# rayanirban/DiffSplitting

Hardware: AMD Instinct MI355X
Metric: sampled images/sec (2000-step 128x128 SR3) (higher is better)
Workload: dtype bf16; 1 GPU; sr_sr3_16_128: GaussianDiffusion.p_sample_loop, 16->128 SR3 UNet (97.8M params), T=2000 linear schedule; one step = UNet forward + posterior update of the batch; batch_per_gpu=16, global_batch=16, image=128x128x3, sample_steps=2000, parallelism=1 independent replicas, final RCCL all-gather, hipgraph=True, streams=1, noise=device Philox4x32-10, weights=random-init, seed 0

## Files before the change

### diffsplitting_amd/csrc/dsx_conv.hip

```cpp
#include "dsx_conv_variants.h"
#include <mutex>

namespace dsx {

int conv_chunk_multiple(int ks) { return conv_cpg(ks); }

static_assert(kIndex.unique, "kVariants: two rows share a key, or a key is outside key_slot's ranges");

static constexpr bool variants_consistent() {
  for (const ConvVariant& a : kVariants) {
    const bool big = a.family != FAM_MFMA || (a.ks == 3 && a.cpg == 2);
    if (a.lds_cap != (big ? kLdsMax : kLdsDefault) || a.block != (a.family == FAM_MFMA ? 256 : 512)) return false;
    for (const ConvVariant& b : kVariants) {
      if (a.tile == b.tile && (a.MB * a.WM != b.MB * b.WM || a.WN * a.NB != b.WN * b.NB)) return false;
      if (a.tile == b.tile && a.family == b.family && (a.WM != b.WM || a.fuses_stats != b.fuses_stats)) return false;
    }
  }
  return true;
}
static_assert(variants_consistent(), "kVariants: wrong LDS limit / block size, or two layouts for one tile");

ConvTileInfo conv_tile_info(int tile, bool ws) {
  for (const ConvVariant& v : kVariants)
    if (v.family == (ws ? FAM_WS : FAM_MFMA) && v.tile == tile) return {32 * v.MB * v.WM, 32 * v.WN * v.NB, v.WM, v.fuses_stats};
  return {0, 0, 0, false};
}

namespace lds_row_was {
constexpr int banked(int rb, int tw_log2) {
  if (tw_log2 == 4) rb = (rb + 255) & ~255;
  else if (tw_log2 == 3) { rb = (rb + 127) & ~127; if (((rb >> 7) & 1) == 0) rb += 128; }
  return rb;
}
constexpr int plain(int ks, int stride, int tw_log2) {
  const int rb = ((((1 << tw_log2) - 1) * stride + ks) * (64 * conv_cpg(ks) + 16) + 15) & ~15;
  return (ks == 1 || stride != 1) ? rb : banked(rb, tw_log2);
}
constexpr int g2(int tw_log2) { return banked(((((1 << tw_log2) - 1) + 3) * (64 * 2 + 16) + 15) & ~15, tw_log2); }
constexpr int c3x3(int tw_log2, int cpg) { return banked(((((1 << tw_log2) - 1) + 3) * (64 * cpg + 16) + 15) & ~15, tw_log2); }
constexpr int c4_1x1(int tw_log2) { return (((1 << tw_log2) * (64 * 4 + 16)) + 15) & ~15; }
constexpr bool same() {
  for (int tw = 0; tw <= 4; ++tw) {
    for (int cpg = 1; cpg <= 4; cpg *= 2)
      if (conv_lds_row(3, 1, tw, cpg) != c3x3(tw, cpg)) return false;
    if (conv_lds_row(3, 1, tw, 1) != plain(3, 1, tw) || conv_lds_row(3, 1, tw, 2) != g2(tw)) return false;
    if (conv_lds_row(3, 2, tw, 1) != plain(3, 2, tw)) return false;
    if (conv_lds_row(1, 1, tw, 2) != plain(1, 1, tw) || conv_lds_row(1, 1, tw, 4) != c4_1x1(tw)) return false;
  }
  return true;
}
static_assert(same(), "conv_lds_row changed a row pitch");
}

hipError_t conv_init() {
  static std::mutex mu;
  static bool done = false;
  std::lock_guard<std::mutex> lock(mu);
  if (done) return hipSuccess;
  for (const ConvVariant& v : kVariants) {
    const hipError_t e = hipFuncSetAttribute((const void*)v.kern, hipFuncAttributeMaxDynamicSharedMemorySize, v.lds_cap);
    if (e != hipSuccess) return e;
  }
  done = true;
  return hipSuccess;
}

}
```

### diffsplitting_amd/csrc/dsx_conv_direct.hip

```cpp
#include "dsx_conv_common.h"

namespace dsx {

template <typename DT>
__global__ __launch_bounds__(256) void k_conv_first(const ConvArgs a) {
  constexpr bool F32 = sizeof(DT) == 4;
  constexpr int ES = (int)sizeof(DT);
  constexpr int KSTEP = F32 ? 2 : 16;
  constexpr int NS16 = 4;
  __shared__ __attribute__((aligned(16))) unsigned char sm[18 * 18 * 7 * 4 + 64 * 4];
  DT* patch = (DT*)sm;
  int* kofft = (int*)(sm + 18 * 18 * 7 * 4);

  const int tid = threadIdx.x, lane = tid & 63;
  const int wave = __builtin_amdgcn_readfirstlane(tid >> 6);
  const int li = lane & 31, lh = lane >> 5;
  const int Cin = a.C0 + a.C1, K = 9 * Cin;
  const int tiles_x = a.Wo >> 4, tiles_y = a.Ho >> 4;
  const int t = blockIdx.x % (tiles_x * tiles_y), b = blockIdx.x / (tiles_x * tiles_y);
  const int ty = t / tiles_x, tx = t - ty * tiles_x;
  const int oy0 = ty * 16, ox0 = tx * 16;
  const int NBLK = (a.Cout + 31) >> 5;

  for (int e = tid; e < 18 * 18 * Cin; e += 256) {
    const int c = e % Cin, pp = e / Cin, px = pp % 18, py = pp / 18;
    const int iy = oy0 + py - 1, ix = ox0 + px - 1;
    DT v = (DT)0.f;
    if (iy >= 0 && iy < a.Hs && ix >= 0 && ix < a.Ws) {
      const size_t pix = ((size_t)b * a.Hs + iy) * a.Ws + ix;
      v = c < a.C0 ? ((const DT*)a.src0)[pix * a.C0 + c] : ((const DT*)a.src1)[pix * a.C1 + (c - a.C0)];
    }
    patch[e] = v;
  }
  if (F32 && tid < 64) {
    const int k = tid < K ? tid : 0;
    const int tap = k / Cin, c = k - tap * Cin;
    kofft[tid] = ((tap / 3) * 18 + (tap % 3)) * Cin + c;
  }
  int koff[F32 ? 1 : NS16 * 8];
  if constexpr (!F32) {
#pragma unroll
    for (int s = 0; s < NS16; ++s)
#pragma unroll
      for (int j = 0; j < 8; ++j) {
        int k = 16 * s + 8 * lh + j;
        if (k >= K) k = 0;
        const int tap = k / Cin, c = k - tap * Cin;
        koff[s * 8 + j] = (((tap / 3) * 18 + (tap % 3)) * Cin + c) * 2;
      }
  }
  uint4 wf[F32 ? 1 : 2 * NS16];
  if constexpr (!F32) {
#pragma unroll
    for (int nb = 0; nb < 2; ++nb)
#pragma unroll
      for (int s = 0; s < NS16; ++s)
        wf[nb * NS16 + s] = nb < NBLK ? ((const uint4*)a.wpack)[(nb * NS16 + s) * 64 + lane] : make_uint4(0u, 0u, 0u, 0u);
  }
  __syncthreads();

  f32x16 acc[2][2];
#pragma unroll
  for (int mb = 0; mb < 2; ++mb)
#pragma unroll
    for (int nb = 0; nb < 2; ++nb)
#pragma unroll
      for (int r = 0; r < 16; ++r) acc[mb][nb][r] = 0.f;

#pragma unroll
  for (int mb = 0; mb < 2; ++mb) {
    const int m = (wave * 2 + mb) * 32 + li;
    const int base = ((m >> 4) * 18 + (m & 15)) * Cin;
    if constexpr (F32) {
      const int nsteps = (K + 1) >> 1;
      const float* wp = (const float*)a.wpack;
      for (int s = 0; s < nsteps; ++s) {
        const float pv = ((const float*)patch)[base + kofft[2 * s + lh]];
#pragma unroll
        for (int nb = 0; nb < 2; ++nb) {
          if (nb < NBLK) acc[mb][nb] = __builtin_amdgcn_mfma_f32_32x32x2f32(wp[(nb * 32 + s) * 64 + lane], pv, acc[mb][nb], 0, 0, 0);
        }
      }
    } else {
      const unsigned char* pb = (const unsigned char*)patch + base * 2;
#pragma unroll
      for (int s = 0; s < NS16; ++s) {
        unsigned w4[4];
#pragma unroll
        for (int q = 0; q < 4; ++q) {
          const unsigned lo = *(const unsigned short*)(pb + koff[s * 8 + 2 * q]);
          const unsigned hi = *(const unsigned short*)(pb + koff[s * 8 + 2 * q + 1]);
          w4[q] = lo | (hi << 16);
        }
        const f32x4_t px = __builtin_bit_cast(f32x4_t, make_uint4(w4[0], w4[1], w4[2], w4[3]));
#pragma unroll
        for (int nb = 0; nb < 2; ++nb)
          if (nb < NBLK) acc[mb][nb] = mfma_step<DT>(wf[nb * NS16 + s], px, acc[mb][nb]);
      }
    }
  }
  (void)KSTEP; (void)ES;

  const int okind = a.out_bf16;
#pragma unroll
  for (int nb = 0; nb < 2; ++nb) {
    const int nbase = nb * 32 + 16 * lh;
    if (nb >= NBLK) continue;
    float s1[16], s2[16];
#pragma unroll
    for (int r = 0; r < 16; ++r) { s1[r] = 0.f; s2[r] = 0.f; }
    const bool live = nbase < a.Cout;
#pragma unroll
    for (int mb = 0; mb < 2; ++mb) {
      const int m = (wave * 2 + mb) * 32 + li;
      const size_t opix = ((size_t)b * a.Ho + (oy0 + (m >> 4))) * a.Wo + (ox0 + (m & 15));
      float x[16], pv[16];
#pragma unroll
      for (int r = 0; r < 16; ++r) { x[r] = acc[mb][nb][r]; pv[r] = 0.f; }
      if (live) {
        if (a.bias) {
#pragma unroll
          for (int j = 0; j < 4; ++j) { const float4 tt = *(const float4*)(a.bias + nbase + 4 * j); pv[4 * j] = tt.x; pv[4 * j + 1] = tt.y; pv[4 * j + 2] = tt.z; pv[4 * j + 3] = tt.w; }
#pragma unroll
          for (int r = 0; r < 16; ++r) x[r] += pv[r];
        }
        store16<true>(a.out, opix * a.out_ld + nbase, x, okind, 16);
#pragma unroll
        for (int r = 0; r < 16; ++r) { const float d = x[r] - pv[r]; s1[r] += d; s2[r] += d * d; }
      }
    }
    if (a.stat_part != nullptr) {
      float w1 = row16_fold(s1, lane), w2 = row16_fold(s2, lane);
      w1 += __shfl_xor(w1, 16, 64);
      w2 += __shfl_xor(w2, 16, 64);
      const int nch = tiles_x * tiles_y * 4, chunk = t * 4 + wave;
      const int n = nbase + row16_fold_reg(li);
      if (li < 16 && n < a.Cout) {
        float* pp = a.stat_part + (((size_t)b * nch + chunk) * a.Cout + n) * 2;
        pp[0] = w1; pp[1] = w2;
      }
    }
  }
}

bool conv_first_applicable(int ks, int stride, const ConvArgs& a, bool gn) {
  const int C = a.C0 + a.C1;
  return ks == 3 && stride == 1 && !a.up && !gn && !a.swish && C >= 1 && C <= 7 && a.Cout >= 16 && a.Cout <= 64 &&
         (a.Cout & 15) == 0 && (a.Ho & 15) == 0 && (a.Wo & 15) == 0 && a.Ho == a.Hs && a.Wo == a.Ws && a.out_ld == a.Cout;
}
hipError_t launch_conv_first(int dtype, const ConvArgs& a, hipStream_t st) {
  const unsigned grid = (unsigned)(a.B * (a.Ho >> 4) * (a.Wo >> 4));
  if (dtype == 1) hipLaunchKernelGGL(k_conv_first<__bf16>, dim3(grid), dim3(256), 0, st, a);
  else if (dtype == 2) hipLaunchKernelGGL(k_conv_first<_Float16>, dim3(grid), dim3(256), 0, st, a);
  else hipLaunchKernelGGL(k_conv_first<float>, dim3(grid), dim3(256), 0, st, a);
  return hipGetLastError();
}

__global__ void k_conv_naive(const NaiveConvArgs na) {
  const ConvArgs& a = na.c;
  const long long total = (long long)a.B * a.Ho * a.Wo * a.Cout;
  const int C = a.C0 + a.C1;
  const int pad = na.ks / 2;
  const int Hi = a.up ? a.Hs * 2 : a.Hs, Wi = a.up ? a.Ws * 2 : a.Ws;
  for (long long idx = blockIdx.x * (long long)blockDim.x + threadIdx.x; idx < total;
       idx += (long long)gridDim.x * blockDim.x) {
    const int n = (int)(idx % a.Cout);
    long long p = idx / a.Cout;
    const int ox = (int)(p % a.Wo); p /= a.Wo;
    const int oy = (int)(p % a.Ho);
    const int b = (int)(p / a.Ho);
    float acc = 0.f;
    for (int dy = 0; dy < na.ks; ++dy) {
      const int iy = oy * na.stride + dy - pad;
      if (iy < 0 || iy >= Hi) continue;
      for (int dx = 0; dx < na.ks; ++dx) {
        const int ix = ox * na.stride + dx - pad;
        if (ix < 0 || ix >= Wi) continue;
        const int sy = a.up ? iy >> 1 : iy, sx = a.up ? ix >> 1 : ix;
        const size_t so = ((size_t)b * a.Hs + sy) * a.Ws + sx;
        const float* w = na.w + (((size_t)n * na.ks + dy) * na.ks + dx) * C;
        for (int c = 0; c < C; ++c) {
          float v = c < a.C0 ? act_load_kind(a.src0, so * a.C0 + c, a.act_bf16)
                             : act_load_kind(a.src1, so * a.C1 + (c - a.C0), a.act_bf16);
          if (a.gn_scale) v = v * a.gn_scale[(size_t)b * C + c] + a.gn_shift[(size_t)b * C + c];
          if (a.swish) v = swish_f(v);
          acc = fmaf(v, w[c], acc);
        }
      }
    }
    const size_t opix = ((size_t)b * a.Ho + oy) * a.Wo + ox;
    float v = acc + (a.bias ? a.bias[n] : 0.f);
    if (a.film) v += a.film[(size_t)b * a.film_bs + n];
    if (a.resid) v += act_load_kind(a.resid, opix * a.resid_ld + n, a.act_bf16);
    if (na.sigmoid_out) v = 1.0f / (1.0f + __expf(-v));
    act_store(a.out, opix * a.out_ld + n, v, a.out_bf16);
  }
}

hipError_t launch_conv_naive(const NaiveConvArgs& a, hipStream_t st) {
  const long long total = (long long)a.c.B * a.c.Ho * a.c.Wo * a.c.Cout;
  long long blocks = (total + 255) / 256;
  if (blocks > 8192) blocks = 8192;
  hipLaunchKernelGGL(k_conv_naive, dim3((unsigned)blocks), dim3(256), 0, st, a);
  return hipGetLastError();
}

}
```

### diffsplitting_amd/csrc/dsx_kernels.h

```cpp
#pragma once
#include <hip/hip_runtime.h>
#include <stdint.h>

namespace dsx {

struct PrefetchArgs {
  const void* base;
  unsigned slice_bytes;
  int nslices;
  unsigned* sink;
};
inline unsigned fastdiv_magic(unsigned d) { return d <= 1 ? 0u : (unsigned)((1ull << 32) / d) + 1u; }
#if defined(__HIPCC__)
__device__ __forceinline__ unsigned fastdiv(unsigned n, unsigned magic) { return magic ? __umulhi(n, magic) : n; }
struct PfAcc { unsigned v[4]; };
__device__ __forceinline__ PfAcc l2_prefetch(const PrefetchArgs& pf, unsigned lin_block, unsigned nblocks_total, int tid, int nthreads) {
  PfAcc acc = {{0u, 0u, 0u, 0u}};
  if (pf.base == nullptr || pf.nslices <= 0) return acc;
  const unsigned label = lin_block & 7u, j = lin_block >> 3, n8 = (nblocks_total + 7u) >> 3;
  const unsigned lines = pf.slice_bytes >> 7;
  const unsigned per = (lines + n8 - 1u) / n8, l0 = j * per;
  const unsigned l1 = l0 + per < lines ? l0 + per : lines;
  const int s0 = pf.nslices < 8 ? (int)(label % (unsigned)pf.nslices) : (int)label;
  const int sstep = pf.nslices < 8 ? pf.nslices : 8;
// ... 85 lines not shown
            ps[u] += ch == 0 ? a.count * p : 0.0;
          }
        }
      }
#pragma unroll
      for (int u = 0; u < 8; ++u) { s += ps[u]; q += pq[u]; }
    }
  };
  const int c_own = c_lo + tid;
  const bool own = tid < cpg;
  const float g_own = own ? a.gamma[c_own] : 0.f, b_own = own ? a.beta[c_own] : 0.f;
  if (n0 > 0) accumulate(a.part0, a.f32_0, n0, a.nchunk0, a.C0, c_lo, a.piv0);
  if (n1 > 0) accumulate(a.part1, a.f32_1, n1, a.nchunk1, a.C1, c_lo + n0 - a.C0, a.piv1);
#pragma unroll
  for (int o = 32; o > 0; o >>= 1) { s += __shfl_xor(s, o, 64); q += __shfl_xor(q, o, 64); }
  if constexpr (NW > 1) {
    if ((tid & 63) == 0) { red[2 * (tid >> 6)] = s; red[2 * (tid >> 6) + 1] = q; }
    __syncthreads();
    s = 0; q = 0;
#pragma unroll
    for (int w = 0; w < NW; ++w) { s += red[2 * w]; q += red[2 * w + 1]; }
  }
  const double n = a.count * cpg;
  const double mean = s / n;
  double var = q / n - mean * mean;
  if (var < 0) var = 0;
  const float rstd = (float)(1.0 / sqrt(var + (double)a.eps));
  const float meanf = (float)mean;
  if (own) {
    const float sc = rstd * g_own;
    a.scale[(size_t)b * C + c_own] = sc;
    a.shift[(size_t)b * C + c_own] = b_own - meanf * sc;
  }
  for (int c = c_lo + tid + NT; c < c_lo + cpg; c += NT) {
    const float sc = rstd * a.gamma[c];
    a.scale[(size_t)b * C + c] = sc;
    a.shift[(size_t)b * C + c] = a.beta[c] - meanf * sc;
  }
}
#endif

struct ConvArgs {
  const void* src0;
  const void* src1;
  int act_bf16;
  int out_bf16;
  int C0, C1;
  int B, Hs, Ws;
  int up;
  int Ho, Wo;
  const float* gn_scale;
  const float* gn_shift;
  int has_gn;
  int swish;
  int stage_mode;
  const void* wpack;
  const float* bias;
  const float* film;
  int film_bs;
  const void* resid;
  int resid_ld;
  void* out;
  int out_ld;
  int Cout;
  int nblocks;
  int kchunks;
  int tw_log2, th_log2, tb_log2;
  int tiles_x, tiles_y, m_tiles, n_tiles;
  int lds_row;
  int cpg;
  int ws_wg_per_n;
  int ws_cpg;
  int xcd_bands;
  int ws_map;
  int ws_nt_log2;
  int ws_per;
  int ws_adv_x, ws_adv_y, ws_adv_b;
  int ws_dpy, ws_dpx;
  unsigned mg_tiles_x, mg_per_img, mg_pw, mg_wpn, mg_per;
  int ws_bigdiv;
  float* stat_part;
  unsigned* handoff_timeouts;
  int ws_direct;
  unsigned long long* stamp;
  int stamp_block;
  int ablate;
  const void* gn_part0; int gn_nchunk0, gn_pf32_0;
  const void* gn_part1; int gn_nchunk1, gn_pf32_1;
  StatPivot gn_piv0, gn_piv1;
  const float* gn_gamma; const float* gn_beta;
  int gn_groups; float gn_eps;
  PrefetchArgs pf;
  int fin_on;
  GnFinArgs fin;
  int ksplit;
  int groups_per_split;
  long long slab_stride;
};

enum ConvTile { TILE_256x128 = 0, TILE_128x128, TILE_64x128, TILE_256x64, TILE_128x64, TILE_64x64, TILE_128x32, TILE_256x32, TILE_COUNT };
struct ConvTileInfo { int BM, BN, WM; bool fuses_stats; };
ConvTileInfo conv_tile_info(int tile, bool ws = false);
int conv_chunk_multiple(int ks);
constexpr int conv_lds_row(int ks, int stride, int tw_log2, int cpg) {
  const int pixb = 64 * cpg + 16;
  const int pw = ((1 << tw_log2) - 1) * stride + ks;
  int rb = (pw * pixb + 15) & ~15;
  if (ks == 1 || stride != 1) return rb;
  if (tw_log2 == 4) rb = (rb + 255) & ~255;
  else if (tw_log2 == 3) { rb = (rb + 127) & ~127; if (((rb >> 7) & 1) == 0) rb += 128; }
  return rb;
}
size_t conv_lds_bytes(int dtype, int tile, int ks, int stride, const ConvArgs& a);
hipError_t launch_conv(int dtype, int tile, int ks, int stride, const ConvArgs& a, hipStream_t st);
size_t conv_ws_lds_bytes(int dtype, int tile, int ks, const ConvArgs& a);
hipError_t launch_conv_ws(int dtype, int tile, int ks, const ConvArgs& a, hipStream_t st);
bool conv_img_applicable(int dtype, int ks, int stride, const ConvArgs& a, bool gn, int gn_groups);
hipError_t launch_conv_img(int dtype, int ks, const ConvArgs& a, hipStream_t st);
bool conv_first_applicable(int ks, int stride, const ConvArgs& a, bool gn);
hipError_t launch_conv_first(int dtype, const ConvArgs& a, hipStream_t st);
hipError_t conv_init();
hipError_t ops_init();

struct NaiveConvArgs {
  ConvArgs c;
  const float* w;
  int ks, stride;
  int sigmoid_out;
};
hipError_t launch_conv_naive(const NaiveConvArgs& a, hipStream_t st);

hipError_t launch_chan_stats(const void* x, int bf16, int B, int HW, int C, int nchunk, double* part,
                             hipStream_t st);
hipError_t launch_gn_finalize(const GnFinArgs& a, hipStream_t st);

struct TembArgs {
  int flavour;
  int B;
  int n_time;
  const float* time;
  const float* table;
  const int* step_ctr;
  int per_sample;
  int inner;
  const float* freq;
  const float* w1; const float* b1;
  const float* w2; const float* b2;
  const float* wf; const float* bf;
  int F;
  float* film;
};
hipError_t launch_temb(const TembArgs& a, hipStream_t st);

struct SplitKReduceArgs {
  const float* slab; int nsplit; long long slab_stride;
  long long M; int N; int HW;
  const float* bias; const float* film; int film_bs;
  const void* resid; int resid_ld;
  void* out;
  int act_bf16;
  float* stat_part;
};
hipError_t launch_splitk_reduce(const SplitKReduceArgs& a, hipStream_t st);

struct AttnArgs {
  const void* q; const void* k; const void* v; int ld;
  void* out; int ldo;
  int storage;
  int B, L, C;
  float div, inv_div;
};
bool attn_supported(int C, int L);
hipError_t launch_attn(const AttnArgs& a, bool col_split, hipStream_t st);

hipError_t launch_nchw_slice_to_nhwc(const float* src, void* dst, int dst_bf16, int B, int C, int ctot, int coff,
                                     int HW, hipStream_t st);
hipError_t launch_nhwc_to_nchw(const float* src, float* dst, int B, int C, int H, int W, hipStream_t st);

constexpr int kUpdateCols = 7;
struct UpdateArgs {
  float* x;
  void* x_act;
  int x_act_kind;
  const float* net;
  float* x0_hist;
  int use_noise;
  const unsigned long long* loop_params;
  const float* tab;
  int n_steps;
  const int* step_ctr;
  int predict_eps, clip;
  int per_sample;
  int B, C, H, W;
  const unsigned long long* sample_ids;
};
hipError_t launch_update(const UpdateArgs& a, hipStream_t st);
constexpr int kStreamRows = 32;
struct StreamIds { unsigned long long subseq[kStreamRows]; };
template <class F>
static inline hipError_t each_stream_chunk(int B, const uint64_t* ids, uint64_t draw, F&& f) {
  for (int b0 = 0; b0 < B; b0 += kStreamRows) {
    StreamIds s{};
    const int rows = B - b0 < kStreamRows ? B - b0 : kStreamRows;
// ... 322 lines not shown
```

### diffsplitting_amd/csrc/dsx_plan.cpp

```cpp
#include "dsx_rt.h"

static std::vector<int> tile_order(const char* e, const std::vector<int>& dflt) {
  if (!*e) return dflt;
  std::vector<int> v;
  for (const char* p = e; *p;) {
    v.push_back(atoi(p));
    while (*p && *p != ',') ++p;
    if (*p == ',') ++p;
  }
  return v;
}

PlanKnobs dsx::read_plan_knobs() {
  PlanKnobs k;
  static const struct { const char* name; int PlanKnobs::*field; } ints[] = {
      {"DSX_FIRST", &PlanKnobs::first}, {"DSX_IMG", &PlanKnobs::img}, {"DSX_WS", &PlanKnobs::ws},
      {"DSX_WS_1X1", &PlanKnobs::ws_1x1}, {"DSX_WS_MIN_GRID", &PlanKnobs::ws_min_grid}, {"DSX_WS_G2", &PlanKnobs::ws_g2},
      {"DSX_WS_G2_MIN64", &PlanKnobs::ws_g2_min64}, {"DSX_WS_G2_MIN128", &PlanKnobs::ws_g2_min128},
      {"DSX_WS_G4_MIN64", &PlanKnobs::ws_g4_min64}, {"DSX_WS_C4", &PlanKnobs::ws_c4},
      {"DSX_WS_C4_MIN", &PlanKnobs::ws_c4_min}, {"DSX_WS_DIRECT", &PlanKnobs::ws_direct}, {"DSX_WS_MAP3", &PlanKnobs::ws_map3},
      {"DSX_XCD_BANDS", &PlanKnobs::xcd_bands}, {"DSX_HOST_FIN", &PlanKnobs::host_fin},
      {"DSX_PREFETCH", &PlanKnobs::prefetch}, {"DSX_PREFETCH_WS", &PlanKnobs::prefetch_ws},
      {"DSX_FUSE_STATS", &PlanKnobs::fuse_stats}, {"DSX_NARROW_G2", &PlanKnobs::narrow_g2},
      {"DSX_MIN_GRID", &PlanKnobs::min_grid}, {"DSX_SPLITK", &PlanKnobs::splitk}, {"DSX_ATTN_CS", &PlanKnobs::attn_cs},
#ifdef DSX_DIAG
      {"DSX_ABLATE", &PlanKnobs::ablate},
#endif
  };
  static const struct { const char* name; std::vector<int> PlanKnobs::*field; } lists[] = {
      {"DSX_TILES_WIDE", &PlanKnobs::tiles_wide}, {"DSX_TILES_NARROW", &PlanKnobs::tiles_narrow},
      {"DSX_TILES_SLIM", &PlanKnobs::tiles_slim}, {"DSX_TILES_WIDE_SPLIT", &PlanKnobs::tiles_wide_split},
      {"DSX_TILES_NARROW_SPLIT", &PlanKnobs::tiles_narrow_split}, {"DSX_TILES_NARROW_G2", &PlanKnobs::tiles_narrow_g2},
      {"DSX_TILES_WS_WIDE", &PlanKnobs::tiles_ws_wide}, {"DSX_TILES_WS_WIDE_1X1", &PlanKnobs::tiles_ws_wide_1x1},
      {"DSX_TILES_WS_WIDE_1X1_RAW", &PlanKnobs::tiles_ws_wide_1x1_raw}, {"DSX_TILES_WS_NARROW", &PlanKnobs::tiles_ws_narrow},
  };
  for (const auto& e : ints)
    if (const char* v = getenv(e.name)) k.*e.field = atoi(v);
  for (const auto& e : lists)
    if (const char* v = getenv(e.name)) k.*e.field = tile_order(v, k.*e.field);
  const char* impl = getenv("DSX_CONV_IMPL");
  k.conv_naive = impl && !strcmp(impl, "naive");
  if (const char* path = getenv("DSX_PLAN_DUMP")) k.plan_dump = path;
  if (const char* se = getenv("DSX_STAMP_OP")) {
    const char* comma = strchr(se, ',');
    k.stamp_op = atoi(se);
    k.stamp_block = comma ? atoi(comma + 1) : 0;
  }
  return k;
}

hipError_t dsx::launch_op(const PlanOp& o, hipStream_t st) {
  switch (o.launcher) {
    case L_CONV_FIRST: return launch_conv_first(o.dtype, o.args.conv, st);
    case L_CONV_IMG: return launch_conv_img(o.dtype, o.ks, o.args.conv, st);
    case L_CONV_WS: return launch_conv_ws(o.dtype, o.tile, o.ks, o.args.conv, st);
    case L_CONV_MFMA: return launch_conv(o.dtype, o.tile, o.ks, o.stride, o.args.conv, st);
    case L_SPLITK_REDUCE: return launch_splitk_reduce(o.args.reduce, st);
    case L_CONV_NAIVE: return launch_conv_naive(o.args.naive, st);
    case L_CHAN_STATS: {
      const ChanStatsArgs& c = o.args.stats;
      return launch_chan_stats(c.x, c.xbf, c.B, c.HW, c.C, c.nchunk, c.part, st);
    }
    case L_GN_FINALIZE: return launch_gn_finalize(o.args.fin, st);
    case L_ATTN: return launch_attn(o.args.attn, o.col_split != 0, st);
  }
  return hipErrorInvalidValue;
}

static int dump_plan(const dsx_exec* ex) {
  static const struct { const char* name; size_t bytes; } L[] = {
      {"conv_first", sizeof(ConvArgs)}, {"conv_img", sizeof(ConvArgs)}, {"conv_ws", sizeof(ConvArgs)},
      {"conv_mfma", sizeof(ConvArgs)}, {"splitk_reduce", sizeof(SplitKReduceArgs)}, {"conv_naive", sizeof(NaiveConvArgs)},
      {"chan_stats", sizeof(ChanStatsArgs)}, {"gn_finalize", sizeof(GnFinArgs)}, {"attn", sizeof(AttnArgs)}};
  FILE* f = fopen(ex->knobs.plan_dump.c_str(), "w");
  if (!f) return fail(DSX_ERR_INVALID, "DSX_PLAN_DUMP: cannot write %s", ex->knobs.plan_dump.c_str());
  for (size_t i = 0; i < ex->ops.size(); ++i) {
    const PlanOp& o = ex->ops[i];
    const char* name = (o.launcher == L_GN_FINALIZE && gn_finalize_is_wide(o.args.fin)) ? "gn_finalize_wide" : L[o.launcher].name;
    fprintf(f, "%zu kind=%d desc=\"%s\" flops=%.17g bytes=%.17g launcher=%s dtype=%d tile=%d ks=%d stride=%d col_split=%d args=",
            i, o.kind, o.desc.c_str(), o.flops, o.bytes, name, o.dtype, o.tile, o.ks, o.stride, o.col_split);
    const unsigned char* p = (const unsigned char*)&o.args;
    for (size_t b = 0; b < L[o.launcher].bytes; ++b) fprintf(f, "%02x", p[b]);
    fputc('\n', f);
  }
  fclose(f);
  return DSX_OK;
}

static int add_op(dsx_exec* ex, int kind, const std::string& desc, double flops, double bytes, Launcher launcher) {
  PlanOp op;
  op.kind = kind; op.desc = desc; op.flops = flops; op.bytes = bytes; op.launcher = launcher;
  ex->ops.push_back(op);
  return (int)ex->ops.size() - 1;
}
static std::string fmt(const char* f, ...) {
  char buf[256];
  va_list ap;
  va_start(ap, f);
  vsnprintf(buf, sizeof buf, f, ap);
// ... 143 lines not shown
    if (wpn > a.m_tiles) wpn = (a.m_tiles + unit - 1) / unit * unit;
  }
  return wpn;
}

static void decide_ws_chunks(const PlanKnobs& k, int dtype, int ks, int tile, ConvArgs& a) {
  auto take = [&](bool wanted, int cpg) {
    ConvArgs t = a;
    t.ws_cpg = cpg; t.lds_row = conv_lds_row(ks, 1, a.tw_log2, cpg);
    if (wanted && conv_ws_lds_bytes(dtype, tile, ks, t) != 0) { a.ws_cpg = cpg; a.lds_row = t.lds_row; }
  };
  if (ks == 3) {
    const int min_chunks = conv_tile_info(tile).BM == 64 ? k.ws_g2_min64 : k.ws_g2_min128;
    take(k.ws_g2 && a.kchunks >= min_chunks, 2);
    take(k.ws_g2 && a.kchunks >= k.ws_g4_min64, 4);
  }
  if (ks == 1) take(k.ws_c4 && a.kchunks >= k.ws_c4_min, 4);
  if (ks == 1 && k.ws_direct && !a.has_gn && !a.swish) {
    ConvArgs t = a;
    t.ws_direct = 1;
    if (conv_ws_lds_bytes(dtype, tile, ks, t) != 0) a.ws_direct = 1;
  }
}

static int decide_ws_startup(const PlanKnobs& k, int ks, ConvArgs& w) {
  w.xcd_bands = k.xcd_bands;
  w.ws_wg_per_n = ws_wg_per_n(w);
  const bool map3 = k.ws_map3 && ks == 1 && w.n_tiles >= 2 && w.n_tiles <= 32;
  if (map3) {
    int wpn3 = std::max(8, (256 / w.n_tiles) / 8 * 8);
    if (wpn3 > w.m_tiles) wpn3 = (w.m_tiles + 7) / 8 * 8;
    w.ws_wg_per_n = wpn3;
  }
  const int NT = w.n_tiles, wpn = w.ws_wg_per_n, per_img = w.tiles_x * w.tiles_y;
  w.ws_map = map3 ? 3 : ((NT <= 8 && 8 % NT == 0 && wpn % (8 / NT) == 0) ? 0 : ((NT % 8) == 0 ? 1 : 2));
  w.ws_nt_log2 = NT <= 8 ? ilog2(NT) : 0;
  w.ws_per = map3 ? NT : (NT >> 3);
  w.ws_adv_x = wpn % w.tiles_x; w.ws_adv_y = (wpn / w.tiles_x) % w.tiles_y; w.ws_adv_b = wpn / per_img;
  const int PW = ((1 << w.tw_log2) - 1) + ks;
  const int upg = 4 * (w.ws_cpg ? w.ws_cpg : conv_chunk_multiple(ks));
  const int pstep = 256 / upg;
  w.ws_dpy = pstep / PW; w.ws_dpx = pstep - w.ws_dpy * PW;
  w.mg_tiles_x = fastdiv_magic((unsigned)w.tiles_x); w.mg_per_img = fastdiv_magic((unsigned)per_img);
  w.mg_pw = fastdiv_magic((unsigned)PW); w.mg_wpn = fastdiv_magic((unsigned)wpn);
  w.mg_per = fastdiv_magic((unsigned)std::max(1, w.ws_per));
  w.ws_bigdiv = ((long long)w.m_tiles + wpn >= 65536 || w.tiles_x >= 65536 || per_img >= 65536) ? 1 : 0;
  auto exact = [](unsigned d, unsigned magic, unsigned nmax) {
    for (unsigned n = 0; n <= nmax; ++n) {
      const unsigned q = magic ? (unsigned)(((unsigned long long)n * magic) >> 32) : n;
      if (q != n / d) return false;
    }
    return true;
  };
  const unsigned grid = (unsigned)(NT * wpn);
  const unsigned nt_max = w.ws_bigdiv ? 0u : (unsigned)(w.m_tiles + wpn);
  if (!exact((unsigned)w.tiles_x, w.mg_tiles_x, grid) || !exact((unsigned)per_img, w.mg_per_img, grid) ||
      !exact((unsigned)PW, w.mg_pw, 255u) || !exact((unsigned)wpn, w.mg_wpn, std::max(grid, nt_max)) ||
      !exact((unsigned)std::max(1, w.ws_per), w.mg_per, grid >> 3))
    return fail(DSX_ERR_INVALID, "planner: fastdiv magic not exact for conv %dx%d @%dx%d", ks, ks, w.Ho, w.Wo);
  return DSX_OK;
}

static int decide_conv(const PlanKnobs& k, int dtype, int norm_groups, const ConvShape& s, ConvChoice& ch) {
  ch = ConvChoice{};
  ch.tile = -1;
  ConvArgs& a = ch.geo;
  a.C0 = s.C0; a.C1 = s.C1;
  a.B = s.B; a.Hs = s.Hs; a.Ws = s.Ws; a.up = s.up ? 1 : 0;
  a.Ho = s.Ho; a.Wo = s.Wo;
  a.swish = s.swish ? 1 : 0;
  a.has_gn = s.has_gn ? 1 : 0;
  a.act_bf16 = dtype;
  a.out_bf16 = s.out_st;
  {
    const int gw = conv_chunk_multiple(s.ks) * (dtype != 0 ? 32 : 16);
    const int um = dtype != 0 ? 7 : 3;
    a.stage_mode = ((a.C0 & um) || (a.C1 & um)) ? 2 : ((a.C1 == 0 || a.C0 % gw == 0) ? 0 : 1);
  }
  a.resid_ld = s.resid_ld; a.out_ld = s.out_ld; a.Cout = s.Cout;
  a.nblocks = s.nblocks; a.kchunks = s.kchunks;
  const int ks = s.ks, stride = s.stride;
  if (!k.conv_naive && k.first && !s.has_film && !s.has_resid && conv_first_applicable(ks, stride, a, s.has_gn)) {
    ch.kernel = CONV_FIRST;
    if (s.want_stats) { ch.stats = STATS_EPILOGUE; ch.stat_nchunk = (a.Ho >> 4) * (a.Wo >> 4) * 4; ch.pivot = PIVOT_BIAS; }
    return DSX_OK;
  }
  if (!k.conv_naive && k.img && !(s.has_resid && (s.resid_ld & 3)) &&
      conv_img_applicable(dtype, ks, stride, a, s.has_gn, norm_groups)) {
    ch.kernel = CONV_IMG;
    ch.gn_in_kernel = s.has_gn;
    if (s.want_stats) { ch.stats = STATS_EPILOGUE; ch.stat_nchunk = 1; }
    return DSX_OK;
  }
  const bool ws_allowed = k.ws && (ks != 1 || k.ws_1x1) && stride == 1 && a.stage_mode == 0;
  if (k.conv_naive || !decide_tile(k, dtype, ks, stride, ws_allowed, a, ch.tile)) {
    if (!s.has_naive)
      return fail(DSX_ERR_INVALID, "no MFMA tile fits conv %dx%d (%dx%d out, B=%d); set DSX_CONV_IMPL=naive", ks, ks,
                  a.Ho, a.Wo, a.B);
    ch.kernel = CONV_NAIVE;
    return DSX_OK;
  }
  const int tile = ch.tile;
  const bool use_ws = ws_allowed && a.cpg != 2 && a.ksplit == 1 && conv_ws_lds_bytes(dtype, tile, ks, a) != 0;
  ch.kernel = a.ksplit > 1 ? CONV_SPLITK : (use_ws ? CONV_WS : (a.cpg == 2 ? CONV_MFMA_G2 : CONV_MFMA));
  if (use_ws) decide_ws_chunks(k, dtype, ks, tile, a);
  const ConvTileInfo ti = conv_tile_info(tile, use_ws);
  if (k.fuse_stats && s.want_stats && ti.fuses_stats &&
      a.ksplit == 1 && a.tb_log2 == 0 && (a.Cout & 15) == 0 && a.out_ld == a.Cout && (a.resid_ld & 7) == 0) {
    ch.stats = STATS_EPILOGUE;
    ch.stat_nchunk = a.tiles_x * a.tiles_y * ti.WM;
  }
  if (a.ksplit > 1 && k.fuse_stats && s.want_stats && a.Cout % 64 == 0 && a.out_ld == a.Cout && (a.Ho * a.Wo) % 16 == 0) {
    ch.stats = STATS_REDUCE;
    ch.stat_nchunk = a.Ho * a.Wo / 16;
    ch.pivot = PIVOT_BIAS_FILM;
  }
  ch.hosts_fin = s.may_host_fin && k.host_fin && use_ws;
  return use_ws ? decide_ws_startup(k, ks, a) : DSX_OK;
}

struct ConvSpec {
  const ConvW* w;
  Tensor x0, x1;
  bool up = false;
  int stride = 1;
  const GnW* gn = nullptr;
  bool has_resid = false;
  bool host_fin = false;
  bool swish = false;
  int film_off = -1;
  const void* resid = nullptr; int resid_ld = 0;
  Tensor out;
  bool want_stats = false;
  bool bias_in_film = false;
};

static bool reserve_stats(dsx_exec* ex, const Tensor& t) {
  StatInfo& si = ex->stats[t.id];
  if (si.planned) return false;
  int nchunk = std::max(1, 512 / ex->B);
  nchunk = std::min(nchunk, std::max(1, t.H * t.W / 16));
  nchunk = std::min(nchunk, 64);
  si.nchunk = nchunk;
  si.part = ws_alloc(ex, (size_t)ex->B * nchunk * t.C * 2 * sizeof(double));
  si.planned = true;
  si.f32 = false;
  return true;
}
static void emit_stats(dsx_exec* ex, const Tensor& t) {
  const StatInfo& si = ex->stats[t.id];
  const int HW = t.H * t.W;
  const int i = add_op(ex, DSX_OP_GN_STATS, fmt("gn_stats C=%d @%dx%d", t.C, t.H, t.W), 0.0,
                       (t.st ? 2.0 : 4.0) * ex->B * HW * t.C, L_CHAN_STATS);
  ChanStatsArgs& c = ex->ops[i].args.stats;
  c.x = t.p; c.xbf = t.st; c.B = ex->B; c.HW = HW; c.C = t.C; c.nchunk = si.nchunk; c.part = (double*)si.part;
}

static float* plan_fused_stats(dsx_exec* ex, const Tensor& t, int nchunk, int C) {
  StatInfo& si = ex->stats[t.id];
  si.nchunk = nchunk;
  si.part = ws_alloc(ex, (size_t)ex->B * nchunk * C * 2 * sizeof(float));
  si.planned = true;
  si.f32 = true;
  return (float*)si.part;
}

// ... 385 lines not shown
```

### diffsplitting_amd/csrc/dsx_rt.h

```cpp
#pragma once
#include <hip/hip_runtime.h>

#include <algorithm>
#include <cmath>
#include <cstdarg>
#include <cstdio>
#include <cstdlib>
#include <cstring>
#include <memory>
#include <string>
#include <utility>
#include <vector>

#include "../../include/dsx.h"
#include "dsx_kernels.h"

using namespace dsx;

namespace dsx {

int fail(int code, const char* fmt, ...);
#define HIP_TRY(expr)                                                                     \
  do {                                                                                    \
    hipError_t e__ = (expr);                                                              \
    if (e__ != hipSuccess)                                                                \
      return fail(DSX_ERR_HIP, "%s failed: %s (%s:%d)", #expr, hipGetErrorString(e__),    \
                  __FILE__, __LINE__);                                                    \
  } while (0)

struct DevBuf {
  void* p = nullptr;
  DevBuf() = default;
  DevBuf(DevBuf&& o) noexcept : p(o.p) { o.p = nullptr; }
  DevBuf& operator=(DevBuf&& o) noexcept { std::swap(p, o.p); return *this; }
  ~DevBuf() { reset(); }
  void reset() { if (p) (void)hipFree(p); p = nullptr; }
  template <class T> T* as() const { return (T*)p; }
  hipError_t alloc(size_t bytes) {
    reset();
    const hipError_t e = hipMalloc(&p, bytes);
    if (e != hipSuccess) p = nullptr;
    return e;
  }
  hipError_t upload(const void* host, size_t bytes) {
    const hipError_t e = alloc(bytes);
    return e != hipSuccess ? e : hipMemcpy(p, host, bytes, hipMemcpyHostToDevice);
  }
};
struct PinnedBuf {
  void* p = nullptr;
  PinnedBuf() = default;
  PinnedBuf(PinnedBuf&& o) noexcept : p(o.p) { o.p = nullptr; }
  PinnedBuf& operator=(PinnedBuf&& o) noexcept { std::swap(p, o.p); return *this; }
  ~PinnedBuf() { reset(); }
  void reset() { if (p) (void)hipHostFree(p); p = nullptr; }
  template <class T> T* as() const { return (T*)p; }
  hipError_t alloc(size_t bytes) {
    reset();
    const hipError_t e = hipHostMalloc(&p, bytes, hipHostMallocDefault);
    if (e != hipSuccess) p = nullptr;
    return e;
  }
};
struct Event {
  hipEvent_t e = nullptr;
  Event() = default;
  Event(Event&& o) noexcept : e(o.e) { o.e = nullptr; }
  Event& operator=(Event&& o) noexcept { std::swap(e, o.e); return *this; }
  ~Event() { reset(); }
  void reset() { if (e) (void)hipEventDestroy(e); e = nullptr; }
  hipError_t create(unsigned flags = hipEventDefault) { reset(); return hipEventCreateWithFlags(&e, flags); }
};
struct Stream {
  hipStream_t s = nullptr;
  Stream() = default;
  Stream(Stream&& o) noexcept : s(o.s) { o.s = nullptr; }
  Stream& operator=(Stream&& o) noexcept { std::swap(s, o.s); return *this; }
  ~Stream() { reset(); }
  void reset() { if (s) (void)hipStreamDestroy(s); s = nullptr; }
  hipError_t create(unsigned flags) { reset(); return hipStreamCreateWithFlags(&s, flags); }
};
struct Graph {
  hipGraph_t graph = nullptr;
  hipGraphExec_t exec = nullptr;
  Graph() = default;
  Graph(Graph&& o) noexcept : graph(o.graph), exec(o.exec) { o.graph = nullptr; o.exec = nullptr; }
  Graph& operator=(Graph&& o) noexcept { std::swap(graph, o.graph); std::swap(exec, o.exec); return *this; }
  ~Graph() { reset(); }
  void reset() {
    if (exec) (void)hipGraphExecDestroy(exec);
    if (graph) (void)hipGraphDestroy(graph);
    exec = nullptr; graph = nullptr;
  }
};

struct PlanKnobs {
  bool conv_naive = false;
  int first = 1;
  int img = 1;
  int ws = 1;
  int ws_1x1 = 1;
  int ws_min_grid = 224;
  int ws_g2 = 1;
  int ws_g2_min64 = 12;
  int ws_g2_min128 = 4;
  int ws_g4_min64 = 16;
  int ws_c4 = 1;
  int ws_c4_min = 8;
  int ws_direct = 1;
  int ws_map3 = 1;
  int xcd_bands = 1;
  int host_fin = 1;
  int prefetch = 1;
  int prefetch_ws = 1;
  int fuse_stats = 1;
  int narrow_g2 = 1;
  int min_grid = 512;
  int splitk = 1;
  int attn_cs = 2;
  int stamp_op = -1;
  int stamp_block = 0;
  std::string plan_dump;
  int ablate = 0;
  std::vector<int> tiles_wide{TILE_128x128, TILE_64x128, TILE_64x64};
  std::vector<int> tiles_narrow{TILE_64x64, TILE_128x64};
  std::vector<int> tiles_slim{TILE_128x32, TILE_64x64, TILE_128x64};
  std::vector<int> tiles_wide_split{TILE_64x128, TILE_128x128, TILE_64x64};
  std::vector<int> tiles_narrow_split{TILE_64x64, TILE_128x64};
  std::vector<int> tiles_narrow_g2{TILE_256x32, TILE_128x32};
  std::vector<int> tiles_ws_wide{TILE_128x128, TILE_64x128};
  std::vector<int> tiles_ws_wide_1x1{TILE_128x128, TILE_64x128};
  std::vector<int> tiles_ws_wide_1x1_raw{TILE_64x128, TILE_128x128};
  std::vector<int> tiles_ws_narrow{TILE_256x64, TILE_128x64, TILE_64x64};
};

struct Param {
  std::string name;
  std::vector<int64_t> shape;
  std::vector<float> host;
  bool set = false;
  int64_t numel() const {
    int64_t n = 1;
    for (auto s : shape) n *= s;
    return n;
  }
};

struct ConvW {
  int pw = -1, pb = -1;
  int cin = 0, cout = 0, ks = 1;
  int kchunks = 0, nblocks = 0;
  void* pack = nullptr;
  void* pack_first = nullptr;
  float* bias = nullptr;
  float* naive = nullptr;
};
struct GnW {
  int pg = -1, pb = -1;
  int C = 0;
  float* gamma = nullptr;
  float* beta = nullptr;
};
struct LinW {
  int pw = -1, pb = -1;
  int in = 0, out = 0;
};

struct Module {
  int kind;
  int section;
  int cin = 0, cout = 0, skip = 0;
  bool attn = false;
  ConvW conv;
  GnW gn1, gn2, gna;
  ConvW conv1, conv2, res, qkv, out;
  bool has_res = false;
  LinW film;
  int film_off = -1;
};

}
// ... 101 lines not shown
```

Before: 3.027 images/s.

## Add persistent double-buffered streaming kernel for the first 3x3 convolution

Adds a persistent variant of the first-layer conv in which each block walks a run of 16x16 tiles. It prefetches the next tile's input through buffer loads into registers while computing the current one, then parks it into a second LDS buffer. Weights and bias are staged once per block in LDS, and the LDS row pitch is picked to reduce bank conflicts. The grid is sized from measured occupancy, which adds launch-time setup and more complex indexing for a layer that is a small part of the UNet.

After: 3.033 images/s, median of 5. About the same (+0.2%).

```diff
diff --git a/diffsplitting_amd/csrc/dsx_conv.hip b/diffsplitting_amd/csrc/dsx_conv.hip
--- a/diffsplitting_amd/csrc/dsx_conv.hip
+++ b/diffsplitting_amd/csrc/dsx_conv.hip
@@ -61,6 +61,8 @@
     const hipError_t e = hipFuncSetAttribute((const void*)v.kern, hipFuncAttributeMaxDynamicSharedMemorySize, v.lds_cap);
     if (e != hipSuccess) return e;
   }
+  const hipError_t e = conv_first_init();
+  if (e != hipSuccess) return e;
   done = true;
   return hipSuccess;
 }
diff --git a/diffsplitting_amd/csrc/dsx_conv_direct.hip b/diffsplitting_amd/csrc/dsx_conv_direct.hip
--- a/diffsplitting_amd/csrc/dsx_conv_direct.hip
+++ b/diffsplitting_amd/csrc/dsx_conv_direct.hip
@@ -1,4 +1,5 @@
 #include "dsx_conv_common.h"
+#include <algorithm>
 
 namespace dsx {
 
@@ -143,12 +144,326 @@
   }
 }
 
+struct FirstStream {
+  int run, total, rp;
+  unsigned mg_cin, mg_rd[2], mg_ce[2];
+};
+
+template <typename DT, bool PAIR, int NBLK>
+__global__ __launch_bounds__(256, 2) void k_conv_first_stream(const ConvArgs a, const FirstStream g) {
+  constexpr bool F32 = sizeof(DT) == 4;
+  constexpr int ES = (int)sizeof(DT), EPD = 4 / ES;
+  constexpr int NS16 = 4;
+  constexpr int NSLOT = F32 ? 10 : 6;
+  constexpr int RPMAX = F32 ? 160 : 96;
+  constexpr int PATCHB = 18 * RPMAX * 4;
+  constexpr unsigned F_L = 1u << 16, F_R = 1u << 17, F_T = 1u << 18, F_B = 1u << 19, F_SKIP = 1u << 20;
+  static_assert(!PAIR || !F32, "dword pairs: 16-bit operands");
+  __shared__ __attribute__((aligned(16))) unsigned char sm[2 * PATCHB + 2 * 64 * 4 + (F32 ? 2 * 32 * 64 * 4 : 2 * NS16 * 64 * 16)];
+  float* bias_s = (float*)(sm + 2 * PATCHB);
+  int* kofft = (int*)(sm + 2 * PATCHB + 256);
+  float* w_s = (float*)(sm + 2 * PATCHB + 512);
+
+  const int tid = threadIdx.x, lane = tid & 63;
+  const int wave = __builtin_amdgcn_readfirstlane(tid >> 6);
+  const int li = lane & 31, lh = lane >> 5;
+  const int C0 = a.C0, C1 = a.C1, Cin = C0 + C1, K = 9 * Cin;
+  const int H = a.Hs, W = a.Ws;
+  const int tiles_x = a.Wo >> 4, tiles_y = a.Ho >> 4, per_img = tiles_x * tiles_y;
+  const int RPB = g.rp * 4, PB = 18 * RPB;
+
+  const int gt0 = (int)blockIdx.x * g.run;
+  const int nt = min(g.run, g.total - gt0);
+  if (nt <= 0) return;
+  int b = gt0 / per_img, ty, tx;
+  { const int t = gt0 - b * per_img; ty = t / tiles_x; tx = t - ty * tiles_x; }
+
+  const int mis0 = (C0 * ES) & 2, mis1 = (C1 * ES) & 2;
+  const int RD0 = (mis0 + 18 * C0 * ES + 3) >> 2, RD1 = C1 ? (mis1 + 18 * C1 * ES + 3) >> 2 : 0;
+  const int NS0 = (18 * RD0 + 255) >> 8, NS1 = (18 * RD1 + 255) >> 8;
+  int gofs[NSLOT];
+  unsigned eaf[NSLOT][EPD];
+#pragma unroll
+  for (int i = 0; i < NSLOT; ++i) {
+    const bool s1 = i >= NS0;
+    const int Cs = s1 ? C1 : C0, RDs = s1 ? RD1 : RD0, mis = s1 ? mis1 : mis0, cb = s1 ? C0 : 0;
+    const int dd = tid + 256 * (s1 ? i - NS0 : i);
+    const bool valid = i < NS0 + NS1 && dd < 18 * RDs;
+    const int py = valid ? (int)fastdiv((unsigned)dd, g.mg_rd[s1 ? 1 : 0]) : 0, jj = dd - py * RDs;
+    gofs[i] = valid ? py * (W * Cs * ES) + jj * 4 - mis : (int)0x80000000;
+#pragma unroll
+    for (int e = 0; e < EPD; ++e) {
+      const int pb = jj * 4 + e * ES - mis;
+      unsigned v = F_SKIP;
+      if (valid && pb >= 0 && pb < 18 * Cs * ES) {
+        const int px = (int)fastdiv((unsigned)pb, g.mg_ce[s1 ? 1 : 0]), c = (pb - px * (Cs * ES)) / ES;
+        v = (unsigned)(py * RPB + (px * Cin + cb + c) * ES) | (px == 0 ? F_L : 0u) | (px == 17 ? F_R : 0u) |
+            (py == 0 ? F_T : 0u) | (py == 17 ? F_B : 0u);
+      }
+      eaf[i][e] = v;
+    }
+  }
+  const __amdgpu_buffer_rsrc_t rs0 = __builtin_amdgcn_make_buffer_rsrc((void*)a.src0, 0, a.B * H * W * C0 * ES, 0x00020000);
+  const __amdgpu_buffer_rsrc_t rs1 = __builtin_amdgcn_make_buffer_rsrc((void*)(a.src1 ? a.src1 : a.src0), 0,
+                                                                       a.src1 ? a.B * H * W * C1 * ES : 0, 0x00020000);
+  unsigned pre[NSLOT];
+  auto load_tile = [&](int tb, int tty, int ttx) {
+    const int opix = (tb * H + tty * 16 - 1) * W + ttx * 16 - 1;
+    const int org0 = opix * (C0 * ES), org1 = opix * (C1 * ES);
+#pragma unroll
+    for (int i = 0; i < NSLOT; ++i) {
+      if (i < NS0) pre[i] = (unsigned)__builtin_amdgcn_raw_buffer_load_b32(rs0, org0 + gofs[i], 0, 0);
+      else if (i < NS0 + NS1) pre[i] = (unsigned)__builtin_amdgcn_raw_buffer_load_b32(rs1, org1 + gofs[i], 0, 0);
+    }
+  };
+  auto border_mask = [&](int tty, int ttx) -> unsigned {
+    return (ttx == 0 ? F_L : 0u) | (ttx == tiles_x - 1 ? F_R : 0u) | (tty == 0 ? F_T : 0u) | (tty == tiles_y - 1 ? F_B : 0u);
+  };
+  auto park_tile = [&](unsigned km, int buf) {
+    unsigned char* dst = sm + buf * PB;
+#pragma unroll
+    for (int i = 0; i < NSLOT; ++i) {
+      if (i >= NS0 + NS1) continue;
+#pragma unroll
+      for (int e = 0; e < EPD; ++e) {
+        const unsigned af = eaf[i][e];
+        if (af & F_SKIP) continue;
+        const unsigned v = (af & km) ? 0u : pre[i];
+        if constexpr (F32) *(unsigned*)(dst + (af & 0xffffu)) = v;
+        else *(unsigned short*)(dst + (af & 0xffffu)) = (unsigned short)(v >> (16 * e));
+      }
+    }
+  };
+
+  load_tile(b, ty, tx);
+
+  if (tid < 64) bias_s[tid] = (a.bias && tid < a.Cout) ? a.bias[tid] : 0.f;
+  const int nsteps32 = (K + 1) >> 1;
+  if constexpr (F32) {
+    if (tid < 64) {
+      const int k = tid < K ? tid : 0;
+      const int tap = (int)fastdiv((unsigned)k, g.mg_cin), c = k - tap * Cin;
+      kofft[tid] = (tap / 3) * RPB + ((tap % 3) * Cin + c) * 4;
+    }
+    const float* wp = (const float*)a.wpack;
+    for (int i = tid; i < 2 * 32 * 64; i += 256)
+      if ((i >> 11) < NBLK && ((i >> 6) & 31) < nsteps32) w_s[i] = wp[i];
+  }
+  unsigned koff[F32 ? 1 : (PAIR ? NS16 * 4 : NS16 * 8)];
+  unsigned dupm = 0;
+  if constexpr (!F32) {
+#pragma unroll
+    for (int s = 0; s < NS16; ++s)
+#pragma unroll
+      for (int j = 0; j < 8; j += (PAIR ? 2 : 1)) {
+        int k = 16 * s + 8 * lh + j;
+        if (k >= K) { k = 0; if (PAIR) dupm |= 1u << (s * 4 + j / 2); }
+        const int tap = (int)fastdiv((unsigned)k, g.mg_cin), c = k - tap * Cin;
+        koff[PAIR ? s * 4 + j / 2 : s * 8 + j] = (unsigned)((tap / 3) * RPB + ((tap % 3) * Cin + c) * 2);
+      }
+  }
+  if constexpr (!F32) {
+    for (int i = tid; i < NBLK * NS16 * 64; i += 256) ((uint4*)w_s)[i] = ((const uint4*)a.wpack)[i];
+  }
+  int pbase[2];
+#pragma unroll
+  for (int mb = 0; mb < 2; ++mb) {
+    const int m = (wave * 2 + mb) * 32 + li;
+    pbase[mb] = (m >> 4) * RPB + (m & 15) * Cin * ES;
+  }
+  park_tile(border_mask(ty, tx), 0);
+
+  const int okind = a.out_bf16;
+  int p = 0;
+  for (int it = 0; it < nt; ++it) {
+    __syncthreads();
+    int nb_ = b, nty = ty, ntx = tx + 1;
+    if (ntx == tiles_x) { ntx = 0; if (++nty == tiles_y) { nty = 0; ++nb_; } }
+    const bool more = it + 1 < nt;
+    if (more) load_tile(nb_, nty, ntx);
+
+    f32x16 acc[2][2];
+#pragma unroll
+    for (int mb = 0; mb < 2; ++mb)
+#pragma unroll
+      for (int nb = 0; nb < 2; ++nb)
+#pragma unroll
+        for (int r = 0; r < 16; ++r) acc[mb][nb][r] = 0.f;
+    const unsigned char* patch = sm + p * PB;
+    if constexpr (F32) {
+#pragma unroll
+      for (int mb = 0; mb < 2; ++mb) {
+        const unsigned char* pb = patch + pbase[mb];
+        for (int s = 0; s < nsteps32; ++s) {
+          const float pv = *(const float*)(pb + kofft[2 * s + lh]);
+#pragma unroll
+          for (int nb = 0; nb < 2; ++nb) {
+            if (nb < NBLK) acc[mb][nb] = __builtin_amdgcn_mfma_f32_32x32x2f32(w_s[(nb * 32 + s) * 64 + lane], pv, acc[mb][nb], 0, 0, 0);
+          }
+        }
+      }
+    } else {
+#pragma unroll
+      for (int s = 0; s < NS16; ++s) {
+        uint4 wf[2];
+#pragma unroll
+        for (int nb = 0; nb < 2; ++nb)
+          wf[nb] = nb < NBLK ? ((const uint4*)w_s)[(nb * NS16 + s) * 64 + lane] : make_uint4(0u, 0u, 0u, 0u);
+#pragma unroll
+        for (int mb = 0; mb < 2; ++mb) {
+          const unsigned char* pb = patch + pbase[mb];
+          unsigned w4[4];
+#pragma unroll
+          for (int q = 0; q < 4; ++q) {
+            if constexpr (PAIR) {
+              const unsigned w = *(const unsigned*)(pb + koff[s * 4 + q]);
+              w4[q] = (dupm >> (s * 4 + q)) & 1u ? (w & 0xffffu) | (w << 16) : w;
+            } else {
+              const unsigned lo = *(const unsigned short*)(pb + koff[s * 8 + 2 * q]);
+              const unsigned hi = *(const unsigned short*)(pb + koff[s * 8 + 2 * q + 1]);
+              w4[q] = lo | (hi << 16);
+            }
+          }
+          const f32x4_t px = __builtin_bit_cast(f32x4_t, make_uint4(w4[0], w4[1], w4[2], w4[3]));
+#pragma unroll
+          for (int nb = 0; nb < 2; ++nb)
+            if (nb < NBLK) acc[mb][nb] = mfma_step<DT>(wf[nb], px, acc[mb][nb]);
+        }
+      }
+    }
+
+    if (more) park_tile(border_mask(nty, ntx), p ^ 1);
+
+    const int oy0 = ty * 16, ox0 = tx * 16, t = ty * tiles_x + tx;
+#pragma unroll
+    for (int nb = 0; nb < 2; ++nb) {
+      const int nbase = nb * 32 + 16 * lh;
+      if (nb >= NBLK) continue;
+      float s1[16], s2[16];
+#pragma unroll
+      for (int r = 0; r < 16; ++r) { s1[r] = 0.f; s2[r] = 0.f; }
+      const bool live = nbase < a.Cout;
+#pragma unroll
+      for (int mb = 0; mb < 2; ++mb) {
+        const int m = (wave * 2 + mb) * 32 + li;
+        const size_t opix = ((size_t)b * a.Ho + (oy0 + (m >> 4))) * a.Wo + (ox0 + (m & 15));
+        float x[16], pv[16];
+#pragma unroll
+        for (int r = 0; r < 16; ++r) { x[r] = acc[mb][nb][r]; pv[r] = 0.f; }
+        if (live) {
+          if (a.bias) {
+#pragma unroll
+            for (int j = 0; j < 4; ++j) { const float4 tt = *(const float4*)(bias_s + nbase + 4 * j); pv[4 * j] = tt.x; pv[4 * j + 1] = tt.y; pv[4 * j + 2] = tt.z; pv[4 * j + 3] = tt.w; }
+#pragma unroll
+            for (int r = 0; r < 16; ++r) x[r] += pv[r];
+          }
+          store16<true>(a.out, opix * a.out_ld + nbase, x, okind, 16);
+#pragma unroll
+          for (int r = 0; r < 16; ++r) { const float d = x[r] - pv[r]; s1[r] += d; s2[r] += d * d; }
+        }
+      }
+      if (a.stat_part != nullptr) {
+        float w1 = row16_fold(s1, lane), w2 = row16_fold(s2, lane);
+        w1 += __shfl_xor(w1, 16, 64);
+        w2 += __shfl_xor(w2, 16, 64);
+        const int nch = per_img * 4, chunk = t * 4 + wave;
+        const int n = nbase + row16_fold_reg(li);
+        if (li < 16 && n < a.Cout) {
+          float* pp = a.stat_part + (((size_t)b * nch + chunk) * a.Cout + n) * 2;
+          pp[0] = w1; pp[1] = w2;
+        }
+      }
+    }
+    b = nb_; ty = nty; tx = ntx; p ^= 1;
+  }
+}
+
 bool conv_first_applicable(int ks, int stride, const ConvArgs& a, bool gn) {
   const int C = a.C0 + a.C1;
   return ks == 3 && stride == 1 && !a.up && !gn && !a.swish && C >= 1 && C <= 7 && a.Cout >= 16 && a.Cout <= 64 &&
          (a.Cout & 15) == 0 && (a.Ho & 15) == 0 && (a.Wo & 15) == 0 && a.Ho == a.Hs && a.Wo == a.Ws && a.out_ld == a.Cout;
 }
+
+static int first_stream_pitch(int Cin, int es) {
+  const int nat = (18 * Cin * es + 3) / 4;
+  int best = nat, best_cost = 1 << 30;
+  for (int rp = nat; rp < nat + 32; ++rp) {
+    int cost = 0;
+    for (int off = 0; off < 4; off += es) {
+      int dw[32];
+      for (int l = 0; l < 32; ++l) dw[l] = (l >> 4) * rp + ((l & 15) * Cin * es + off) / 4;
+      for (int bank = 0; bank < 32; ++bank) {
+        int distinct = 0;
+        for (int l = 0; l < 32; ++l) {
+          if ((dw[l] & 31) != bank) continue;
+          bool seen = false;
+          for (int m = 0; m < l; ++m) seen = seen || dw[m] == dw[l];
+          if (!seen) ++distinct;
+        }
+        if (distinct > 1) cost += distinct - 1;
+      }
+    }
+    if (cost < best_cost) { best_cost = cost; best = rp; }
+  }
+  return best;
+}
+static bool first_stream_ok(const ConvArgs& a, int es) {
+  int slots = 0;
+  for (int cs : {a.C0, a.C1}) slots += cs ? (18 * ((((cs * es) & 2) + 18 * cs * es + 3) >> 2) + 255) >> 8 : 0;
+  if (slots > (es == 4 ? 10 : 6)) return false;
+  const long long px = (long long)a.B * a.Hs * a.Ws;
+  if (px * a.C0 * es >= (1LL << 30) || px * a.C1 * es >= (1LL << 30)) return false;
+  if (((uintptr_t)a.src0 & 3) || ((uintptr_t)a.src1 & 3)) return false;
+  return a.C1 == 0 || a.src1 != nullptr;
+}
+typedef void (*FirstStreamKernel)(const ConvArgs, const FirstStream);
+template <typename DT> static FirstStreamKernel first_stream_kernel_of(bool pair, int nblk) {
+  if constexpr (sizeof(DT) == 4) return nblk == 2 ? k_conv_first_stream<DT, false, 2> : k_conv_first_stream<DT, false, 1>;
+  else if (pair) return nblk == 2 ? k_conv_first_stream<DT, true, 2> : k_conv_first_stream<DT, true, 1>;
+  else return nblk == 2 ? k_conv_first_stream<DT, false, 2> : k_conv_first_stream<DT, false, 1>;
+}
+static FirstStreamKernel first_stream_kernel(int dtype, bool pair, int nblk) {
+  return dtype == 1 ? first_stream_kernel_of<__bf16>(pair, nblk)
+                    : (dtype == 2 ? first_stream_kernel_of<_Float16>(pair, nblk) : first_stream_kernel_of<float>(false, nblk));
+}
+static int g_first_resident[3][2][2];
+hipError_t conv_first_init() {
+  int dev = 0, cus = 0;
+  hipError_t e = hipGetDevice(&dev);
+  if (e == hipSuccess) e = hipDeviceGetAttribute(&cus, hipDeviceAttributeMultiprocessorCount, dev);
+  for (int dtype = 0; dtype < 3; ++dtype)
+    for (int pair = 0; pair < (dtype ? 2 : 1); ++pair)
+      for (int nblk = 1; nblk <= 2 && e == hipSuccess; ++nblk) {
+        int per_cu = 0;
+        e = hipOccupancyMaxActiveBlocksPerMultiprocessor(&per_cu, (const void*)first_stream_kernel(dtype, pair != 0, nblk), 256, 0);
+        g_first_resident[dtype][pair][nblk - 1] = cus * per_cu;
+      }
+  return e;
+}
+static hipError_t launch_first_stream(int dtype, const ConvArgs& a, hipStream_t st) {
+  const bool pair = dtype != 0 && ((a.C0 + a.C1) & 1) == 0;
+  const int nblk = a.Cout > 32 ? 2 : 1;
+  const int resident = g_first_resident[dtype][pair ? 1 : 0][nblk - 1];
+  FirstStream g;
+  g.total = a.B * (a.Ho >> 4) * (a.Wo >> 4);
+  g.run = std::max(a.first_stream, resident > 0 ? (g.total + resident - 1) / resident : 1);
+  const int es = dtype == 0 ? 4 : 2;
+  g.rp = first_stream_pitch(a.C0 + a.C1, es);
+  g.mg_cin = fastdiv_magic((unsigned)(a.C0 + a.C1));
+  for (int s = 0; s < 2; ++s) {
+    const int cs = s ? a.C1 : a.C0;
+    g.mg_rd[s] = fastdiv_magic((unsigned)((((cs * es) & 2) + 18 * cs * es + 3) >> 2));
+    g.mg_ce[s] = fastdiv_magic((unsigned)(cs * es));
+  }
+  const unsigned grid = (unsigned)((g.total + g.run - 1) / g.run);
+  void* args[] = {(void*)&a, (void*)&g};
+  (void)hipLaunchKernel((const void*)first_stream_kernel(dtype, pair, nblk), dim3(grid), dim3(256), args, 0, st);
+  return hipGetLastError();
+}
 hipError_t launch_conv_first(int dtype, const ConvArgs& a, hipStream_t st) {
+  if (a.first_stream > 0 && first_stream_ok(a, dtype == 0 ? 4 : 2)) {
+    return launch_first_stream(dtype, a, st);
+  }
   const unsigned grid = (unsigned)(a.B * (a.Ho >> 4) * (a.Wo >> 4));
   if (dtype == 1) hipLaunchKernelGGL(k_conv_first<__bf16>, dim3(grid), dim3(256), 0, st, a);
   else if (dtype == 2) hipLaunchKernelGGL(k_conv_first<_Float16>, dim3(grid), dim3(256), 0, st, a);
diff --git a/diffsplitting_amd/csrc/dsx_kernels.h b/diffsplitting_amd/csrc/dsx_kernels.h
--- a/diffsplitting_amd/csrc/dsx_kernels.h
+++ b/diffsplitting_amd/csrc/dsx_kernels.h
@@ -191,6 +191,7 @@
   float* stat_part;
   unsigned* handoff_timeouts;
   int ws_direct;
+  int first_stream;
   unsigned long long* stamp;
   int stamp_block;
   int ablate;
@@ -228,6 +229,7 @@
 hipError_t launch_conv_img(int dtype, int ks, const ConvArgs& a, hipStream_t st);
 bool conv_first_applicable(int ks, int stride, const ConvArgs& a, bool gn);
 hipError_t launch_conv_first(int dtype, const ConvArgs& a, hipStream_t st);
+hipError_t conv_first_init();
 hipError_t conv_init();
 hipError_t ops_init();
 
diff --git a/diffsplitting_amd/csrc/dsx_plan.cpp b/diffsplitting_amd/csrc/dsx_plan.cpp
--- a/diffsplitting_amd/csrc/dsx_plan.cpp
+++ b/diffsplitting_amd/csrc/dsx_plan.cpp
@@ -14,7 +14,7 @@
 PlanKnobs dsx::read_plan_knobs() {
   PlanKnobs k;
   static const struct { const char* name; int PlanKnobs::*field; } ints[] = {
-      {"DSX_FIRST", &PlanKnobs::first}, {"DSX_IMG", &PlanKnobs::img}, {"DSX_WS", &PlanKnobs::ws},
+      {"DSX_FIRST", &PlanKnobs::first}, {"DSX_FIRST_STREAM", &PlanKnobs::first_stream}, {"DSX_IMG", &PlanKnobs::img}, {"DSX_WS", &PlanKnobs::ws},
       {"DSX_WS_1X1", &PlanKnobs::ws_1x1}, {"DSX_WS_MIN_GRID", &PlanKnobs::ws_min_grid}, {"DSX_WS_G2", &PlanKnobs::ws_g2},
       {"DSX_WS_G2_MIN64", &PlanKnobs::ws_g2_min64}, {"DSX_WS_G2_MIN128", &PlanKnobs::ws_g2_min128},
       {"DSX_WS_G4_MIN64", &PlanKnobs::ws_g4_min64}, {"DSX_WS_C4", &PlanKnobs::ws_c4},
@@ -324,6 +324,7 @@
   const int ks = s.ks, stride = s.stride;
   if (!k.conv_naive && k.first && !s.has_film && !s.has_resid && conv_first_applicable(ks, stride, a, s.has_gn)) {
     ch.kernel = CONV_FIRST;
+    a.first_stream = std::max(0, k.first_stream);
     if (s.want_stats) { ch.stats = STATS_EPILOGUE; ch.stat_nchunk = (a.Ho >> 4) * (a.Wo >> 4) * 4; ch.pivot = PIVOT_BIAS; }
     return DSX_OK;
   }
diff --git a/diffsplitting_amd/csrc/dsx_rt.h b/diffsplitting_amd/csrc/dsx_rt.h
--- a/diffsplitting_amd/csrc/dsx_rt.h
+++ b/diffsplitting_amd/csrc/dsx_rt.h
@@ -97,6 +97,7 @@
 struct PlanKnobs {
   bool conv_naive = false;
   int first = 1;
+  int first_stream = 2;
   int img = 1;
   int ws = 1;
   int ws_1x1 = 1;
```
